# rpng/open_vins

Measured on AMD Instinct MI355X. Metric: MSCKF features/sec per EKF update (30-clone state), higher is better.
Workload: dtype f64; 1 GPU; BASELINE.json configs[2]: 2-camera radtan rig, 30-clone window, 2000 MSCKF features/update, N=248, D=208, online cam extrinsic+intrinsic calib + IMU intrinsics in the state, FEJ; features_total=2000, features_this_rank=2000, clones=30, cameras=2, state_dim=248, measurements_total=100362, parallelism=single GPU

## Files before the change

open_vins_amd/csrc/api_context.inc:

```
using namespace ovg;

static thread_local std::string g_err = "";
static int set_err(int code, const std::string &msg) {
  g_err = msg;
  return code;
}

#define HIPCHK(expr)                                                                                         \
  do {                                                                                                       \
    hipError_t _e = (expr);                                                                                  \
    if (_e != hipSuccess) {                                                                                  \
      return set_err(OVGPU_ERR_HIP, std::string(#expr) + " -> " + hipGetErrorString(_e) + " (" __FILE__ ":" + \
                                        std::to_string(__LINE__) + ")");                                     \
    }                                                                                                        \
  } while (0)

namespace {

struct AllocCount {
  std::atomic<int64_t> n{0}, bytes{0};
  void add(size_t b) { n.fetch_add(1, std::memory_order_relaxed), bytes.fetch_add((int64_t)b, std::memory_order_relaxed); }
  void sub(size_t b) { n.fetch_sub(1, std::memory_order_relaxed), bytes.fetch_sub((int64_t)b, std::memory_order_relaxed); }
};
struct DeviceAlloc {
// ... 262 lines not shown
  std::vector<int32_t> h_offsets;
  std::vector<int64_t> h_row_off;

  DevBuf<double> Hbig, gate_ws, Rws, Mt, Aaug, Yaug, dx;
  DevView<int32_t> flags;
  int W = 1;
  int64_t rows_per_node = 128;
  int tsqr_last_W = 0;
  int64_t tsqr_last_rpn = 0;
  int tsqr_last_leaf = -1;
  int tsqr_last_tree = 0;
  int tsqr_last_qh = 0;
  DevBuf<QrTreeNode> tree_nodes, tree_nodes2;
  int tree_G2 = 0;
  Stream stream2;
  Event ev_rows;
  bool gram_il = true;
  bool gram_blocks_only = false;
  bool fuse_chol_inputs = true;
  Event ev_fork, ev_join;
  DevBuf<int32_t> leaf_flags;
  int tree_overlap = -1;
  bool tree_nodes_overlap = false, tree_nodes2_overlap = false;
  DevBuf<int32_t> tree_flags;
  DevBuf<int32_t> tree_err;
  int tree_G = 0;
  bool tree_pipelined = true;
  int compress_gram = 1;
  DevBuf<double> gram_part, gram_G, gram_rho, Yaug2, Lw;
  double prior_pivot_tol = 1e-13;
  int last_route = OVGPU_COMPRESS_GRAM;
  bool whiten = true;
  bool gram_is_whitened = false;
  bool prior_on_side = false;
  int featy_skip = 0;
  DevBuf<double> fs_tq;
  DevBuf<int32_t> fs_inst;
  DevBuf<int32_t> fs_inst64;
  int inst64_D = 0;
  int feat_classes = 0;
  int64_t feat_class_batches = 0;
  int feat_class_attempt = 0;
  int last_feat_classes = 0;
  int last_class_features[4] = {0, 0, 0, 0};
  DevBuf<double> featyb_ws;
  DevBuf<double> slyb_rows, slyb_V, slyb_hq;
  DevBuf<int32_t> slyb_minfo, slyb_inst;
  int featy_big = 0;
  bool no_feat_kernel = false;
  bool raw_enable = true;
  bool gram_read_ahead = true;
  int gram_waves = 8;
  bool featy_chains = true;
  int raw_work_const = 12;
  bool raw_veto = false;
  bool raw_one_region = false;
  bool raw_cols_ok = false;
  bool raw_tables_ok = false;
  int raw_j0 = 0;
  int raw_ncls = 0, raw_ntc[RAW_MAXCLS + 1] = {0}, raw_ld[RAW_MAXCLS + 1] = {0}, raw_rcol[RAW_MAXCLS + 1] = {0};
  int64_t raw_base[RAW_MAXCLS + 1] = {0}, raw_rows[RAW_MAXCLS + 1] = {0};
  std::vector<uint8_t> h_cls_of_clone;
  DevBuf<uint8_t> cls_of_clone;
  DevBuf<int32_t> raw_featbase, raw_dst, raw_runs;
  DevBuf<double> Hraw;
  DevBuf<gram::GramRegionWG> gram_wg;
  int gram_wg_n = 0, gram_wg_tiles = 0;
  gram::GramRegionSum raw_rs;
  bool last_stack_raw = false;
  DevView<int32_t> feat_counter;
  DevBuf<int32_t> fs_minfo, fs_meas_feat, fs_pos;
  DevBuf<int32_t> fs_slots;
  std::vector<int32_t> h_order;
  std::vector<uint16_t> h_cc;
  DevBuf<double> fs_rows, fs_V, fs_z, fs_w;
  void *comm = nullptr;
  struct LoopComm *loop = nullptr;
  int comm_rank = 0, comm_world = 1;
  DevBuf<double> comm_buf;
  DevView<int32_t> chol_prog;
  DevBuf<int32_t> ctrl;
  unsigned ctrl_clean = 0;
  unsigned ctrl_pre = 0;
  DevBuf<double> chol_uinv;
  DevBuf<double> chol_wide_A, chol_wide_Y;
  bool chol_wide = true;
  int64_t chol_wide_count = 0;
  int gram_wide = 0;
  int gram_wide_on = 0;
  int64_t gram_wide_updates = 0;
  int gram_wide_attempt = 0;
  int mode_a_wide = 0;
  int mode_a_wide_on = 0;
  int64_t mode_a_wide_compressions = 0;
  int slam_mode_a = 0;
  int slam_mode_a_on = 0;
  int64_t slam_mode_a_compressions = 0;
  int mode_a_panel = 0;
  int mode_a_panel_on = 0;
  int64_t mode_a_panel_compressions = 0;
  DevBuf<double> pchol_dots;
  DevBuf<double> uinv_tiles;
  PinBuf<double> h_tri;
  int chol_slot = 0;
  bool no_chol_pipe = false;
  int tri_waves = 0;
// ... 213 lines not shown
```

open_vins_amd/csrc/api_debug.inc:

```
int ovgpu_debug_option(ovgpu_ctx *c, const char *name, int64_t value, int64_t *old_value) {
  if (!c || !name) return set_err(OVGPU_ERR_INVALID, "null argument");
  const std::string n(name);
  if (n == "chol_follow_spin_limit") {
    if (old_value) *old_value = c->chol_spin_limit;
    if (value >= 0) c->chol_spin_limit = (int)std::min<int64_t>(value, 1 << 30);
  } else if (n == "slam_chunked_fail_chunk") {
    if (old_value) *old_value = c->chunk_fail_inject;
    c->chunk_fail_inject = value >= 0 ? (int)std::min<int64_t>(value, 1 << 20) : -1;
  } else if (n == "slam_chunked_fallbacks") {
    if (old_value) *old_value = c->chunk_fallbacks;
    if (value >= 0) c->chunk_fallbacks = value;
  } else if (n == "delayed_init_fused") {
    if (old_value) *old_value = c->init_fused;
    if (value >= 0) c->init_fused = (int)std::min<int64_t>(value, 2);
  } else if (n == "delayed_init_fused_steps") {
    if (old_value) *old_value = c->init_fused_steps;
    if (value >= 0) c->init_fused_steps = value;
  } else if (n == "delayed_init_rows_steps") {
    if (old_value) *old_value = c->init_rows_steps;
    if (value >= 0) c->init_rows_steps = value;
  } else if (n == "delayed_init_fused_long") {
    if (old_value) *old_value = c->init_fused_long;
    if (value >= 0) c->init_fused_long = value != 0 ? 1 : 0;
  } else if (n == "delayed_init_long_steps") {
// ... 25 lines not shown
    if (value >= 0) c->anchored_fast = value != 0;
  } else if (n == "slam_fused") {
    if (old_value) *old_value = c->slam_fused;
    if (value >= 0) c->slam_fused = (int)std::min<int64_t>(value, 3);
  } else if (n == "slam_fused_big") {
    if (old_value) *old_value = c->slam_fused_big;
    if (value >= 0) c->slam_fused_big = (int)std::min<int64_t>(value, 1);
  } else if (n == "slam_fused_batches") {
    if (old_value) *old_value = c->slam_fused_batches;
    if (value >= 0) c->slam_fused_batches = value;
  } else if (n == "gram_blocks_only") {
    if (old_value) *old_value = c->gram_blocks_only ? 1 : 0;
    if (value >= 0) c->gram_blocks_only = value != 0;
  } else if (n == "stage_timing_period") {
    if (old_value) *old_value = c->timing_period;
    if (value >= 1) c->timing_period = (int)value, c->timing_seq = 0;
  } else if (n == "fuse_chol_inputs") {
    if (old_value) *old_value = c->fuse_chol_inputs ? 1 : 0;
    if (value >= 0) c->fuse_chol_inputs = value != 0;
  } else if (n == "featy_big") {
    if (old_value) *old_value = c->featy_big;
    if (value >= 0) c->featy_big = (int)value;
  } else if (n == "upload_kernel") {
    if (old_value) *old_value = c->up.use_kernel;
    if (value >= 0) c->up.use_kernel = c->down.use_kernel = value != 0;
  } else if (n == "upload_arena_bytes") {
    if (old_value) *old_value = (int64_t)c->up.capacity();
    if (value >= 64) c->up.want = (size_t)std::min<int64_t>(value, (int64_t)1 << 30);
  } else if (n == "upload_bypasses") {
    if (old_value) *old_value = c->up.bypasses;
    if (value >= 0) c->up.bypasses = value;
  } else if (n == "layout_every_update") {
    if (old_value) *old_value = c->layout_every_update;
    if (value >= 0) c->layout_every_update = value != 0;
  } else if (n == "tri_waves") {
    if (old_value) *old_value = c->tri_waves;
    if (value >= 0 && value <= 16) c->tri_waves = (int)value;
  } else if (n == "featy_skip") {
#ifdef OVG_FEAT_ABLATE
    if (old_value) *old_value = c->featy_skip;
    if (value >= 0) c->featy_skip = (int)value;
#else
    return set_err(OVGPU_ERR_INVALID, "featy_skip: ablation switches exist in a developer build only (-DOVG_FEAT_ABLATE)");
#endif
  } else if (n == "gram_read_ahead") {
    if (old_value) *old_value = c->gram_read_ahead ? 1 : 0;
    if (value >= 0) c->gram_read_ahead = value != 0;
  } else if (n == "gram_waves") {
    if (old_value) *old_value = c->gram_waves;
    if (value >= 0) {
      if (value != 4 && value != 8) return set_err(OVGPU_ERR_INVALID, "gram_waves: 4 or 8");
      c->gram_waves = (int)value;
    }
  } else if (n == "featy_chains") {
    if (old_value) *old_value = c->featy_chains ? 1 : 0;
    if (value >= 0) c->featy_chains = value != 0;
  } else if (n == "raw_work_const") {
    if (old_value) *old_value = c->raw_work_const;
    if (value >= 0) c->raw_work_const = (int)value;
  } else if (n == "last_stack_raw") {
    if (old_value) *old_value = c->last_stack_raw ? 1 : 0;
  } else if (n == "raw_gram_tile_rows") {
    int64_t t = 0;
    if (c->raw_tables_ok)
      for (int k = 0; k <= RAW_NEG; k++) t += c->raw_rows[k] * (int64_t)(c->raw_ntc[k] * (c->raw_ntc[k] + 1) / 2);
    if (old_value) *old_value = t;
  } else if (n == "stack_is_f32") {
    if (old_value) *old_value = c->stack_is_f32 ? 1 : 0;
  } else if (n == "last_feature_kernel") {
    if (old_value) *old_value = c->last_feat_kernel;
  } else if (n == "feat_classes") {
    if (old_value) *old_value = c->feat_classes;
    if (value >= 0) c->feat_classes = (int)std::min<int64_t>(value, 1);
  } else if (n == "feat_class_batches") {
    if (old_value) *old_value = c->feat_class_batches;
    if (value >= 0) c->feat_class_batches = value;
  } else if (n == "last_feature_classes") {
    if (old_value) *old_value = c->last_feat_classes;
  } else if (n.size() == 21 && n.compare(0, 20, "last_class_features_") == 0 && n[20] >= '0' && n[20] <= '3') {
    if (old_value) *old_value = c->last_class_features[n[20] - '0'];
  } else if (n == "last_gram_kernel") {
    if (old_value) *old_value = c->last_gram_kernel;
  } else if (n == "last_gram_workgroups") {
    if (old_value) *old_value = c->last_gram_workgroups;
  } else if (n == "last_factor_kernel") {
    if (old_value) *old_value = c->last_factor_kernel;
  } else if (n == "last_unwhiten_kernel") {
    if (old_value) *old_value = c->last_unwhiten_kernel;
  } else if (n == "chol_wide") {
    if (old_value) *old_value = c->chol_wide ? 1 : 0;
    if (value >= 0) c->chol_wide = value != 0;
  } else if (n == "chol_wide_factorisations") {
    if (old_value) *old_value = c->chol_wide_count;
    if (value >= 0) c->chol_wide_count = value;
  } else if (n == "gram_wide") {
    if (old_value) *old_value = c->gram_wide;
    if (value >= 0) c->gram_wide = (int)std::min<int64_t>(value, 1);
  } else if (n == "gram_wide_updates") {
    if (old_value) *old_value = c->gram_wide_updates;
  } else if (n == "mode_a_wide") {
    if (old_value) *old_value = c->mode_a_wide;
    if (value >= 0) c->mode_a_wide = (int)std::min<int64_t>(value, 1);
  } else if (n == "mode_a_wide_compressions") {
    if (old_value) *old_value = c->mode_a_wide_compressions;
  } else if (n == "mode_a_panel") {
    if (old_value) *old_value = c->mode_a_panel;
// ... 209 lines not shown
```

open_vins_amd/csrc/api_pipeline.inc:

```
static int enqueue_triangulate(ovgpu_ctx *c, const double *seed_pA = nullptr, const int32_t *seed_anchor = nullptr) {
  const Batch b = batch_of(c);
  if (b.F == 0) return OVGPU_OK;
  TriParams p;
  p.seed_pA = seed_pA, p.seed_anchor = seed_anchor, p.anchor_pre = c->anchor_pre.p;
  p.F = b.F, p.C = c->C, p.K = c->K;
  p.meas_offsets = b.meas_offsets, p.meas_cc = b.meas_cc, p.uvn = b.uvn, p.tab_cc = c->tab_cc.p;
  p.p_FinA = b.pA, p.p_FinG = b.pG, p.anchor_meas = c->anchor.p, p.status = b.status;
  p.opt = c->dopt;
  const size_t lds = (size_t)c->K * c->C * 12 * sizeof(double);
  if (lds > (size_t)c->lds_limit) {
    return set_err(OVGPU_ERR_CAPACITY, "k_triangulate: the pose table of K = " + std::to_string(c->K) + " cameras x C = " + std::to_string(c->C) + " clones (96 bytes a pair, " +
                                           std::to_string(lds) + " bytes) exceeds the LDS limit of " + std::to_string(c->lds_limit) + " bytes");
  }
  int wpb = c->tri_waves;
  if (wpb == 0) {
    wpb = 4;
    const int room = c->num_cu - 6;
    for (int w = 4; w <= 8 && room > 0; w *= 2) {
      const int blocks = (b.F + w - 1) / w;
      if (blocks <= room) {
        if (4 * blocks >= 3 * room) wpb = w;
        break;
      }
    }
// ... 317 lines not shown
static int enqueue_gram_factor(ovgpu_ctx *c);
static int gram_blk_row_shares(const ovgpu_ctx *c, int NT, int64_t nchunks) {
  int shares = c->num_cu;
  if (NT > gram::GR_NT_BLK) shares = std::max(1, c->num_cu / (gram::GR_NT_WIDE / gram::GB_T * (gram::GR_NT_WIDE / gram::GB_T + 1) / 2));
  return (int)std::max<int64_t>(1, std::min<int64_t>(shares, nchunks));
}
static size_t gram_part_doubles(const ovgpu_ctx *c, int NT, int64_t nchunks) {
  const size_t G = (size_t)std::max<int64_t>(1, std::min<int64_t>(c->num_cu, nchunks));
  size_t need = NT <= gram::GR_NT_BLK ? G * (size_t)(NT * (NT + 1) / 2) * 256 : 0;
  if (NT > gram::GR_NT || c->gram_fp32) {
    const size_t NB = (size_t)(NT + gram::GB_T - 1) / gram::GB_T, pairs = NB * (NB + 1) / 2;
    need = std::max(need, pairs * (size_t)gram_blk_row_shares(c, NT, nchunks) * gram::GB_T * gram::GB_T * 256);
  }
  return need;
}
static int gram_route_tile_cap(const ovgpu_ctx *c) { return c->gram_wide_on >= 1 && c->whiten && !c->gram_fp32 ? gram::GR_NT_WIDE : gram::GR_NT_BLK; }
static int mode_a_tile_cap(const ovgpu_ctx *c) { return c->mode_a_wide_on >= 1 && c->whiten && !c->gram_fp32 ? gram::GR_NT_WIDE : gram::GR_NT_BLK; }
constexpr int MODE_A_PANEL_MIN_NT = 17;
static bool mode_a_panel_factor(const ovgpu_ctx *c, int NTf) { return c->mode_a_panel_on >= 1 && NTf >= MODE_A_PANEL_MIN_NT && NTf <= gram::GR_NT_BLK; }
static int enqueue_compress_gram(ovgpu_ctx *c, bool factor = true) {
  const int D = c->D, LD = c->LD, NT = (LD + 15) / 16, NP = NT * (NT + 1) / 2, LG = 16 * NT;
  const int64_t rows_total = batch_of(c).rows_total;
  const int64_t nchunks = (rows_total + gram::GR_ROWS - 1) / gram::GR_ROWS;
  const int G = (int)std::max<int64_t>(1, std::min<int64_t>(c->num_cu, nchunks));
  if (NT <= gram::GR_NT_BLK) HIPCHK(c->gram_part.reserve((size_t)G * NP * 256));
  HIPCHK(c->gram_G.reserve((size_t)LG * LG));
  if (c->stack_is_f32) {
    const int LDF = c->stack_ldf, NTM = LDF / 32, P = gram32::gram32_parts(NTM), slots = P * gram32::G32_NW * gram32::G32_MAXT;
    if (c->gram32_ntm != NTM || c->gram32_P != P) {
      std::vector<int32_t> tab((size_t)slots);
      gram32::gram32_tile_table(NTM, P, tab.data());
      HIPCHK(c->gram32_tiles.reserve((size_t)slots));
      HIPCHK(hipMemcpyAsync(c->gram32_tiles.p, tab.data(), sizeof(int32_t) * slots, hipMemcpyHostToDevice, c->stream));
      HIPCHK(upload_sync(c, c->stream));
      c->gram32_ntm = NTM, c->gram32_P = P;
    }
    const int64_t by_rows = (rows_total + gram32::G32_ROWS_WG - 1) / gram32::G32_ROWS_WG;
    const int64_t by_cus = std::min<int64_t>((2 * c->num_cu + P - 1) / P, (rows_total + 127) / 128);
    const int Gw = (int)std::max<int64_t>(1, std::max(by_rows, by_cus));
    HIPCHK(c->gram32_part.reserve((size_t)P * Gw * gram32::G32_NW * gram32::G32_MAXT * 1024));
    gram32::Gram32Params q;
    q.H = c->Hbig32.p, q.part = c->gram32_part.p, q.tiles = c->gram32_tiles.p, q.rows_total = rows_total, q.LDF = LDF, q.LD = LD;
    hipLaunchKernelGGL(with_max_lds<gram32::k_gram_f32>(c), dim3(Gw, P), dim3(gram32::G32_NTH), gram32::gram32_lds_bytes(LDF), c->stream, q);
    hipLaunchKernelGGL(gram32::k_gram_f32_reduce, dim3(slots, 4), dim3(256), 0, c->stream, (const int32_t *)c->gram32_tiles.p, Gw,
                       (const float *)c->gram32_part.p, c->gram_G.p, LG);
    HIPCHK(hipGetLastError());
    c->last_gram_kernel = 5, c->last_gram_workgroups = Gw;
    return factor ? set_err(OVGPU_ERR_CAPACITY, "the fp32 Gram variant feeds the on-device update only") : OVGPU_OK;
  }
  if (c->last_stack_raw) {
    HIPCHK(c->gram_part.reserve((size_t)std::max(c->gram_wg_tiles, 1) * 256));
    const int waves = c->gram_read_ahead ? c->gram_waves : 4;
    const auto kern = !c->gram_read_ahead ? with_max_lds<gram::k_gram_regions<false>>(c)
                      : waves == 8        ? with_max_lds<gram::k_gram_regions<true, 8>>(c)
                                          : with_max_lds<gram::k_gram_regions<true>>(c);
    hipLaunchKernelGGL(kern, dim3(c->gram_wg_n), dim3(64 * waves), gram::gram_lds_bytes(), c->stream, (const double *)c->Hraw.p, (const gram::GramRegionWG *)c->gram_wg.p,
                       c->gram_part.p);
    hipLaunchKernelGGL(gram::k_gram_regions_reduce, dim3(NP, 256 / gram::RR_E), dim3(gram::RR_E * gram::RR_G), 0, c->stream, NT, D, c->raw_rs,
                       (const gram::GramRegionWG *)c->gram_wg.p, c->gram_wg_n, (const double *)c->gram_part.p, c->gram_G.p);
    HIPCHK(hipGetLastError());
    c->last_gram_kernel = 4;
    return factor ? enqueue_gram_factor(c) : OVGPU_OK;
  }
  gram::GramParams g;
  g.LD = LD, g.NT = NT, g.rows_total = rows_total, g.H = c->Hbig.p, g.part = c->gram_part.p;
  if (NT == gram::GR_NT + 7 && !c->gram_fp32 && !c->gram_blocks_only) {
    const int Gw = G;
    hipLaunchKernelGGL(with_max_lds<gram::k_gram_wide_top<7>>(c), dim3(Gw), dim3(256), gram::gram_wide_top_lds_bytes(), c->stream, g);
    hipLaunchKernelGGL(with_max_lds<gram::k_gram_wide_win<7>>(c), dim3(Gw), dim3(256), gram::gram_lds_bytes(), c->stream, g);
    hipLaunchKernelGGL(gram::k_gram_reduce, dim3(NP), dim3(1024), 0, c->stream, NT, Gw, c->gram_part.p, c->gram_G.p);
    HIPCHK(hipGetLastError());
    c->last_gram_kernel = 3;
    return factor ? enqueue_gram_factor(c) : OVGPU_OK;
  }
  if (NT > gram::GR_NT || c->gram_fp32) {
    const int NB = (NT + gram::GB_T - 1) / gram::GB_T, pairs = NB * (NB + 1) / 2;
    const int Gb = gram_blk_row_shares(c, NT, nchunks);
    HIPCHK(c->gram_part.reserve((size_t)pairs * Gb * gram::GB_T * gram::GB_T * 256));
    g.part = c->gram_part.p;
    if (!c->gram_fp32) hipLaunchKernelGGL(with_max_lds<gram::k_gram_blk<false>>(c), dim3(Gb, pairs), dim3(256), gram::gram_blk_lds_bytes(), c->stream, g, NB);
    else hipLaunchKernelGGL(with_max_lds<gram::k_gram_blk<true>>(c), dim3(Gb, pairs), dim3(256), gram::gram_blk_lds_bytes() / 2, c->stream, g, NB);
    hipLaunchKernelGGL(gram::k_gram_blk_reduce, dim3(gram::GB_T * gram::GB_T, pairs), dim3(256), 0, c->stream, NB, NT, Gb, c->gram_part.p, c->gram_G.p);
    HIPCHK(hipGetLastError());
    c->last_gram_kernel = 2, c->last_gram_workgroups = Gb;
    return factor ? enqueue_gram_factor(c) : OVGPU_OK;
  }
  switch ((NT + 1) / 2) {
  case 1: launch_gram<2>(c, G, g, c->stream, c->gram_il); break;
  case 2: launch_gram<4>(c, G, g, c->stream, c->gram_il); break;
  case 3: launch_gram<6>(c, G, g, c->stream, c->gram_il); break;
  case 4: launch_gram<8>(c, G, g, c->stream, c->gram_il); break;
  case 5: launch_gram<10>(c, G, g, c->stream, c->gram_il); break;
  case 6: launch_gram<12>(c, G, g, c->stream, c->gram_il); break;
  case 7: launch_gram<14>(c, G, g, c->stream, c->gram_il); break;
  default:
    if (NT == 15) launch_gram<15>(c, G, g, c->stream, c->gram_il);
    else launch_gram<16>(c, G, g, c->stream, c->gram_il);
    break;
  }
  hipLaunchKernelGGL(gram::k_gram_reduce, dim3(NP), dim3(1024), 0, c->stream, NT, G, c->gram_part.p, c->gram_G.p);
  HIPCHK(hipGetLastError());
  c->last_gram_kernel = 1;
  return factor ? enqueue_gram_factor(c) : OVGPU_OK;
}

static int enqueue_gram_factor(ovgpu_ctx *c) {
  const int D = c->D, LD = c->LD, LG = 16 * ((LD + 15) / 16);
// ... 809 lines not shown
```

open_vins_amd/csrc/api_state.inc:

```

const char *ovgpu_last_error(void) { return g_err.c_str(); }

void ovgpu_default_options(ovgpu_options *o) {
  if (!o) return;
  std::memset(o, 0, sizeof(*o));
  o->chi2_multipler = 5.0, o->sigma_pix = 1.0;
  o->triangulate_1d = 0, o->refine_features = 1, o->max_runs = 5;
  o->init_lamda = 1e-3, o->max_lamda = 1e10, o->min_dx = 1e-6, o->min_dcost = 1e-6, o->lam_mult = 10;
  o->min_dist = 0.10, o->max_dist = 60, o->max_baseline = 40, o->max_cond_number = 10000;
  o->do_fej = 1, o->do_calib_camera_pose = 1, o->do_calib_camera_intrinsics = 1;
  o->feat_rep_msckf = OVGPU_REP_GLOBAL_3D;
}

double ovgpu_chi2_quantile_95(int dof) { return chi2_quantile_95(dof); }
int ovgpu_abi_version(void) { return OVGPU_ABI_VERSION; }

static int init_context(ovgpu_ctx *c, const ovgpu_options *opts, int device) {
  c->device = device;
  c->opts = *opts;
  hipDeviceProp_t prop;
  HIPCHK(hipGetDeviceProperties(&prop, device));
  c->num_cu = prop.multiProcessorCount > 0 ? prop.multiProcessorCount : 256;
  c->lds_limit = (int)std::min<size_t>(prop.sharedMemPerBlock, 160 * 1024);
  HIPCHK(hipStreamCreateWithFlags(&c->stream.h, hipStreamNonBlocking));
// ... 590 lines not shown
  if (!c->raw_enable || !c->raw_cols_ok || F <= 0 || M <= 0 || n <= 0) return OVGPU_OK;
  std::vector<int32_t> fb((size_t)F * RAW_MAXCLS, 0);
  int64_t run[RAW_MAXCLS + 1] = {0};
  for (int f = 0; f < F; f++) {
    int cnt[RAW_MAXCLS] = {0};
    for (int i = b.h_offsets[f]; i < b.h_offsets[f + 1]; i++) cnt[c->h_cls_of_clone[anchor_clone(cc[i])]]++;
    int below = 0;
    for (int k = 0; k < n; k++) {
      fb[(size_t)f * RAW_MAXCLS + k] = (int32_t)(run[k] - 2 * below);
      run[k] += 2 * cnt[k], below += cnt[k];
    }
  }
  run[RAW_NEG] = (int64_t)4 * F;
  int64_t total = 0;
  double work[RAW_MAXCLS + 1] = {0}, work_sum = 0;
  int live = 0;
  for (int k = 0; k <= RAW_NEG; k++) {
    if (k >= n && k != RAW_NEG) {
      c->raw_rows[k] = 0, c->raw_base[k] = total;
      continue;
    }
    if (run[k] >= ((int64_t)1 << RAW_CLS_SHIFT)) return OVGPU_OK;
    c->raw_rows[k] = run[k], c->raw_base[k] = total;
    total += run[k] * c->raw_ld[k];
    work[k] = (double)run[k] * (0.5 * c->raw_ntc[k] * (c->raw_ntc[k] + 1) + (double)c->raw_work_const);
    work_sum += work[k], live += run[k] > 0;
  }
  HIPCHK(c->Hraw.reserve((size_t)std::max<int64_t>(total, 1)));
  HIPCHK(c->raw_featbase.reserve(fb.size()));
  HIPCHK(c->raw_dst.reserve((size_t)M));
  HIPCHK(c->raw_runs.reserve((size_t)F * feat::FY_RUNREC * 4));
  HIPCHK(c->up.put(c->raw_featbase.p, fb.data(), sizeof(int32_t) * fb.size()));
  const int G = std::max(c->num_cu, live);
  int wgs[RAW_MAXCLS + 1] = {0}, given = 0;
  for (int k = 0; k <= RAW_NEG; k++)
    if (c->raw_rows[k] > 0) wgs[k] = std::max(1, (int)std::floor(work[k] / work_sum * (G - live)) + 1), given += wgs[k];
  for (int k = RAW_NEG; given > G && k >= 0; k = k > 0 ? k - 1 : RAW_NEG)
    if (wgs[k] > 1) wgs[k]--, given--;
  std::vector<gram::GramRegionWG> tab;
  int tiles = 0;
  c->raw_rs.n = 0;
  for (int k = 0; k <= RAW_NEG; k++) {
    if (wgs[k] == 0) continue;
    const int64_t nchunks = (c->raw_rows[k] + gram::GR_ROWS - 1) / gram::GR_ROWS;
    const int w = (int)std::min<int64_t>(wgs[k], nchunks);
    {
      const int q = c->raw_rs.n++;
      c->raw_rs.ntc[q] = c->raw_ntc[k], c->raw_rs.rcol[q] = c->raw_rcol[k];
    }
    for (int j = 0; j < w; j++) {
      gram::GramRegionWG r;
      r.ntc = c->raw_ntc[k], r.ld = c->raw_ld[k], r.rcol = c->raw_rcol[k], r.pad = 0;
      if (r.ld > 16 * r.ntc) return set_err(OVGPU_ERR_INVALID, "raw_stack_layout: a region's row stride exceeds its tile columns");
      r.h_off = c->raw_base[k], r.rows = c->raw_rows[k];
      r.chunk_begin = (int)((nchunks * j) / w), r.chunk_end = (int)((nchunks * (j + 1)) / w);
      r.part_tile = tiles, r.region = (c->raw_rs.n - 1) | (k == RAW_NEG ? 16 : 0);
      tiles += r.ntc * (r.ntc + 1) / 2;
      tab.push_back(r);
    }
  }
  c->gram_wg_n = (int)tab.size(), c->gram_wg_tiles = tiles;
  HIPCHK(c->gram_wg.reserve(tab.size()));
  HIPCHK(c->up.put(c->gram_wg.p, tab.data(), sizeof(gram::GramRegionWG) * tab.size()));
  c->raw_tables_ok = true;
  return OVGPU_OK;
}

static int begin_feature_batch(ovgpu_ctx *c, int F, int M, const int32_t *offsets) {
  c->have_feats = false, c->tri_readable = false;
  c->raw_tables_ok = false;
  int m_max = 0;
  for (int f = 0; f < F; f++) {
    const int m = offsets[f + 1] - offsets[f];
    if (m < 0) return set_err(OVGPU_ERR_INVALID, "meas_offsets not monotone");
    m_max = std::max(m_max, m);
  }
  c->F = F, c->M = M, c->m_max = m_max;
  c->have_feat_sigma = c->have_feat_mult = false;
  c->h_feat_lm.clear(), c->h_feat_rep.clear();
  c->h_offsets.assign(offsets, offsets + (F > 0 ? F + 1 : 0));
  if (F == 0) c->h_offsets.assign(1, 0);

  const int need = std::max(500, 2 * m_max + 1);
  if ((int)c->h_chi2_table.size() < need) {
    const int old = (int)c->h_chi2_table.size();
    c->h_chi2_table.resize(need, 0.0);
    for (int i = std::max(old, 1); i < need; i++) c->h_chi2_table[i] = chi2_quantile_95(i);
  }
  c->chi2_table_len = (int)c->h_chi2_table.size();
  HIPCHK(c->chi2_table.reserve(c->chi2_table_len));

  HIPCHK(c->meas_offsets.reserve(F + 1));
  HIPCHK(c->meas_cc.reserve(M));
  HIPCHK(c->uv.reserve((size_t)2 * M));
  HIPCHK(c->uvn.reserve((size_t)2 * M));
  HIPCHK(c->pA.reserve((size_t)3 * F));
  HIPCHK(c->pG.reserve((size_t)3 * F));
  HIPCHK(c->chi2.reserve(F));
  HIPCHK(c->chi2_thr.reserve(F));
  HIPCHK(c->anchor.reserve(F));
  HIPCHK(c->anchor_pre.reserve(F));
  HIPCHK(c->status.reserve(F));

  std::vector<int32_t> order(std::max(F, 1), 0);
  track_order(offsets, F, m_max, order.data());
  c->h_order.assign(order.begin(), order.begin() + F);
// ... 66 lines not shown
```

open_vins_amd/csrc/k_gram.h:

```cpp
#pragma once
#include <hip/hip_runtime.h>
#include <stdint.h>
#include <type_traits>
#include <utility>

namespace ovg {
namespace gram {

typedef double d4 __attribute__((ext_vector_type(4)));

constexpr int GR_ROWS = 32;
constexpr int GR_LS = 272;
constexpr int GR_NT = 16;
constexpr int GR_NT_BLK = 24;
constexpr int GR_NT_WIDE = 32;

struct GramParams {
  int LD, NT;
  int64_t rows_total;
  const double *H;
  double *part;
};

__host__ __device__ inline int pair_index(int NT, int ti, int tj) { return ti * NT - (ti * (ti - 1)) / 2 + (tj - ti); }
// ... 384 lines not shown
        __builtin_amdgcn_sched_barrier(0);
#ifdef OVG_GRAM_PROF
        GRAM_T(w0)
        __builtin_amdgcn_s_waitcnt(0xC07F | ((NU - 1) << 8));
        GRAM_T(w1)
        prof_wait += w1 - w0;
#endif
      }
      static_for(std::make_integer_sequence<int, NS>{}, [&](auto sc) {
        constexpr int s = decltype(sc)::value;
        constexpr bool ahead = ks < 7 && s < NU, slot = s < SL && (ks & 3) * SL + s < NQ;
        if constexpr (s < N) {
          constexpr int ti = D::row_of(T0 + s), tj = D::col_of(T0 + s);
          GRAM_MFMA(bb[ks & 1][ti], bb[ks & 1][tj], acc[s]);
        }
        if constexpr (ahead || slot) __builtin_amdgcn_sched_barrier(0);
        if constexpr (ahead) {
          constexpr int j = D::nth_col(W, s);
          bb[(ks + 1) & 1][j] = rowp[4 * GR_LS + 16 * j];
        }
        if constexpr (slot) {
          constexpr int q = (ks & 3) * SL + s;
          if constexpr (ks < 4) put(nxt, q);
          else fetch1(q);
        }
        if constexpr (ahead || slot) __builtin_amdgcn_sched_barrier(0);
      });
      __builtin_amdgcn_sched_barrier(0);
    });
    left_v = left_f;
#ifdef OVG_GRAM_PROF
    GRAM_T(b0)
#endif
    asm volatile("s_waitcnt lgkmcnt(0)\n\ts_barrier" ::: "memory");
#ifdef OVG_GRAM_PROF
    GRAM_T(b1)
    prof_bar += b1 - b0;
#endif
  }
#ifdef OVG_GRAM_PROF
  GRAM_T(prof_t2)
  if (lane == 0) {
    long long *o = gram_prof_buf + ((size_t)(blockIdx.x & 1023) * 8 + W) * 8;
    o[3] = prof_t1 - prof_t0, o[4] = prof_t2 - prof_t1, o[5] = prof_wait, o[6] = prof_bar;
  }
#endif
#pragma unroll
  for (int s = 0; s < N; s++) {
    double2 *o = reinterpret_cast<double2 *>(p.part + (size_t)(T0 + s) * 256) + lane;
    o[0] = double2{acc[s][0], acc[s][1]}, o[64] = double2{acc[s][2], acc[s][3]};
  }
}

template <int NTC, bool PF, int NW> __device__ __forceinline__ void gram_region_body(const GramParams &p, double *gram_lds, int tid, int lane, int wave, int cb, int ce) {
  if constexpr (NW == 8) {
    switch (wave) {
    case 0: gram_w8<0, NTC>(p, gram_lds, tid, lane, cb, ce); break;
    case 1: gram_w8<1, NTC>(p, gram_lds, tid, lane, cb, ce); break;
    case 2: gram_w8<2, NTC>(p, gram_lds, tid, lane, cb, ce); break;
    case 3: gram_w8<3, NTC>(p, gram_lds, tid, lane, cb, ce); break;
    case 4: gram_w8<4, NTC>(p, gram_lds, tid, lane, cb, ce); break;
    case 5: gram_w8<5, NTC>(p, gram_lds, tid, lane, cb, ce); break;
    case 6: gram_w8<6, NTC>(p, gram_lds, tid, lane, cb, ce); break;
    default: gram_w8<7, NTC>(p, gram_lds, tid, lane, cb, ce); break;
    }
  } else {
    d4 acc[GR_ACC];
#pragma unroll
    for (int i = 0; i < GR_ACC; i++) acc[i] = d4{0, 0, 0, 0};
    switch (wave) {
    case 0: gram_il_loop<0, NTC, true, PF>(p, gram_lds, tid, lane, cb, ce, acc), gram_put<0, true>(p.part, NTC, lane, acc); break;
    case 1: gram_il_loop<1, NTC, true, PF>(p, gram_lds, tid, lane, cb, ce, acc), gram_put<1, true>(p.part, NTC, lane, acc); break;
    case 2: gram_il_loop<2, NTC, true, PF>(p, gram_lds, tid, lane, cb, ce, acc), gram_put<2, true>(p.part, NTC, lane, acc); break;
    default: gram_il_loop<3, NTC, true, PF>(p, gram_lds, tid, lane, cb, ce, acc), gram_put<3, true>(p.part, NTC, lane, acc); break;
    }
  }
}
template <bool PF, int NW = 4> __global__ void __launch_bounds__(64 * NW) k_gram_regions(const double *H, const GramRegionWG *tab, double *part) {
  static_assert(NW == 4 || (NW == 8 && PF), "the eight-wavefront form reads ahead");
  extern __shared__ double gram_lds[];
  const int tid = threadIdx.x, lane = tid & 63, wave = tid >> 6;
  const GramRegionWG r = tab[blockIdx.x];
#ifdef OVG_GRAM_PROF
  const long long prof_w0 = wall_clock64();
  GRAM_T(prof_c0)
#endif
  for (int i = tid, w = 16 * r.ntc - r.ld; i < 2 * GR_ROWS * w; i += 64 * NW) gram_lds[(i / w) * GR_LS + r.ld + i % w] = 0.0;
  __syncthreads();
#ifdef OVG_GRAM_PROF
  GRAM_T(prof_c1)
#endif
  GramParams p;
  p.LD = r.ld, p.NT = r.ntc, p.rows_total = r.rows, p.H = H + r.h_off, p.part = part + (size_t)r.part_tile * 256;
  switch (r.ntc) {
  case 4: gram_region_body<4, PF, NW>(p, gram_lds, tid, lane, wave, r.chunk_begin, r.chunk_end); break;
  case 6: gram_region_body<6, PF, NW>(p, gram_lds, tid, lane, wave, r.chunk_begin, r.chunk_end); break;
  case 8: gram_region_body<8, PF, NW>(p, gram_lds, tid, lane, wave, r.chunk_begin, r.chunk_end); break;
  case 10: gram_region_body<10, PF, NW>(p, gram_lds, tid, lane, wave, r.chunk_begin, r.chunk_end); break;
  case 12: gram_region_body<12, PF, NW>(p, gram_lds, tid, lane, wave, r.chunk_begin, r.chunk_end); break;
  case 14: gram_region_body<14, PF, NW>(p, gram_lds, tid, lane, wave, r.chunk_begin, r.chunk_end); break;
  default: gram_region_body<15, PF, NW>(p, gram_lds, tid, lane, wave, r.chunk_begin, r.chunk_end); break;
  }
#ifdef OVG_GRAM_PROF
  __builtin_amdgcn_s_waitcnt(0x0070);
  GRAM_T(prof_c2)
  if (lane == 0) {
    long long *o = gram_prof_buf + ((size_t)(blockIdx.x & 1023) * 8 + wave) * 8;
    o[0] = prof_w0, o[1] = wall_clock64(), o[2] = prof_c1 - prof_c0, o[7] = (prof_c2 - prof_c1) - o[3] - o[4];
  }
#endif
}

struct GramRegionSum {
  int32_t n;
  int32_t ntc[9], rcol[9];
};
constexpr int RR_E = 64, RR_G = 16, RR_U = 16;
__global__ void __launch_bounds__(RR_E *RR_G) k_gram_regions_reduce(int NT, int D, GramRegionSum rs, const GramRegionWG *__restrict__ tab, int total, const double *__restrict__ part,
                                                                        double *__restrict__ G) {
  __shared__ int eoff[9][RR_E];
  __shared__ double tot[RR_G][RR_E];
  const int LG = 16 * NT;
  const int idx = blockIdx.x, e = threadIdx.x & (RR_E - 1), t = RR_E * blockIdx.y + e;
  const int grp = __builtin_amdgcn_readfirstlane(threadIdx.x / RR_E);
  int ti = 0, rem = idx;
  while (rem >= NT - ti) rem -= NT - ti, ti++;
  const int tj = ti + rem;
  const int q = 2 * (t >> 7) + (t & 1), lane = (t >> 1) & 63;
  const int i = 16 * ti + 4 * q + (lane >> 4), j = 16 * tj + (lane & 15);
  if (grp < rs.n) {
    const int rc = rs.rcol[grp], ntc = rs.ntc[grp];
    int li = i == D ? rc : (i < rc && i < D ? i : -1), lj = j == D ? rc : (j < rc && j < D ? j : -1);
    int off = -1;
    if (li >= 0 && lj >= 0) {
      if ((li >> 4) > (lj >> 4)) {
        const int x = li;
        li = lj, lj = x;
      }
      const int lq = (li & 15) >> 2, llane = 16 * (li & 3) + (lj & 15);
      off = pair_index(ntc, li >> 4, lj >> 4) * 256 + (lq >> 1) * 128 + 2 * llane + (lq & 1);
    }
    eoff[grp][e] = off;
  }
  __syncthreads();
  double s = 0.0;
  for (int base = 0; base < total; base += RR_G * RR_U) {
    int ptile[RR_U], reg[RR_U];
#pragma unroll
    for (int u = 0; u < RR_U; u++) {
      const int f = base + grp + RR_G * u, fc = f < total ? f : total - 1;
      ptile[u] = tab[fc].part_tile, reg[u] = f < total ? tab[fc].region : -1;
    }
    double a[RR_U];
    bool ok[RR_U];
// ... 552 lines not shown
```

Baseline: 2.973 million features/s.

## Stage Gram input tiles into LDS with direct global-to-LDS loads in a ring

Adds an eight-wavefront Gram kernel variant that copies raw Jacobian chunks from global memory straight into a multi-slot LDS ring buffer using global_load_lds, then synchronises with vmcnt-based barriers. The aim is to overlap the next chunks' loads with MFMA work and skip the register round-trip of staging through VGPRs. Padding columns now read from a shared zero slot instead of zeroing LDS pad regions. It becomes the default and adds layout checks for even base and row counts, which could reject layouts that were accepted before.

```diff
diff --git a/open_vins_amd/csrc/api_context.inc b/open_vins_amd/csrc/api_context.inc
--- a/open_vins_amd/csrc/api_context.inc
+++ b/open_vins_amd/csrc/api_context.inc
@@ -338,6 +338,7 @@
   bool gram_read_ahead = true;
   int gram_waves = 8;
   bool featy_chains = true;
+  int gram_stage_dma = 1;
   int raw_work_const = 12;
   bool raw_veto = false;
   bool raw_one_region = false;
diff --git a/open_vins_amd/csrc/api_debug.inc b/open_vins_amd/csrc/api_debug.inc
--- a/open_vins_amd/csrc/api_debug.inc
+++ b/open_vins_amd/csrc/api_debug.inc
@@ -101,6 +101,13 @@
       if (value != 4 && value != 8) return set_err(OVGPU_ERR_INVALID, "gram_waves: 4 or 8");
       c->gram_waves = (int)value;
     }
+  } else if (n == "gram_stage_dma") {
+    if (old_value) *old_value = c->gram_stage_dma;
+    if (value >= 0) {
+      if (value == 2) return set_err(OVGPU_ERR_INVALID, "gram_stage_dma: the padded image (2) is not built");
+      if (value > 1) return set_err(OVGPU_ERR_INVALID, "gram_stage_dma: 0 or 1");
+      c->gram_stage_dma = (int)value;
+    }
   } else if (n == "featy_chains") {
     if (old_value) *old_value = c->featy_chains ? 1 : 0;
     if (value >= 0) c->featy_chains = value != 0;
diff --git a/open_vins_amd/csrc/api_pipeline.inc b/open_vins_amd/csrc/api_pipeline.inc
--- a/open_vins_amd/csrc/api_pipeline.inc
+++ b/open_vins_amd/csrc/api_pipeline.inc
@@ -393,7 +393,7 @@
     HIPCHK(c->gram_part.reserve((size_t)std::max(c->gram_wg_tiles, 1) * 256));
     const int waves = c->gram_read_ahead ? c->gram_waves : 4;
     const auto kern = !c->gram_read_ahead ? with_max_lds<gram::k_gram_regions<false>>(c)
-                      : waves == 8        ? with_max_lds<gram::k_gram_regions<true, 8>>(c)
+                      : waves == 8        ? (c->gram_stage_dma == 1 ? with_max_lds<gram::k_gram_regions<true, 8, 1>>(c) : with_max_lds<gram::k_gram_regions<true, 8>>(c))
                                           : with_max_lds<gram::k_gram_regions<true>>(c);
     hipLaunchKernelGGL(kern, dim3(c->gram_wg_n), dim3(64 * waves), gram::gram_lds_bytes(), c->stream, (const double *)c->Hraw.p, (const gram::GramRegionWG *)c->gram_wg.p,
                        c->gram_part.p);
diff --git a/open_vins_amd/csrc/api_state.inc b/open_vins_amd/csrc/api_state.inc
--- a/open_vins_amd/csrc/api_state.inc
+++ b/open_vins_amd/csrc/api_state.inc
@@ -666,6 +666,8 @@
       gram::GramRegionWG r;
       r.ntc = c->raw_ntc[k], r.ld = c->raw_ld[k], r.rcol = c->raw_rcol[k], r.pad = 0;
       if (r.ld > 16 * r.ntc) return set_err(OVGPU_ERR_INVALID, "raw_stack_layout: a region's row stride exceeds its tile columns");
+      if ((c->raw_base[k] & 1) || (c->raw_rows[k] & 1)) return set_err(OVGPU_ERR_INVALID, "raw_stack_layout: a region's base or row count is no multiple of two doubles");
+      if (r.ld <= 16 * (r.ntc - 2)) return set_err(OVGPU_ERR_INVALID, "raw_stack_layout: a region's rows end before its last two tile columns");
       r.h_off = c->raw_base[k], r.rows = c->raw_rows[k];
       r.chunk_begin = (int)((nchunks * j) / w), r.chunk_end = (int)((nchunks * (j + 1)) / w);
       r.part_tile = tiles, r.region = (c->raw_rs.n - 1) | (k == RAW_NEG ? 16 : 0);
diff --git a/open_vins_amd/csrc/k_gram.h b/open_vins_amd/csrc/k_gram.h
--- a/open_vins_amd/csrc/k_gram.h
+++ b/open_vins_amd/csrc/k_gram.h
@@ -460,8 +460,165 @@
   }
 }
 
-template <int NTC, bool PF, int NW> __device__ __forceinline__ void gram_region_body(const GramParams &p, double *gram_lds, int tid, int lane, int wave, int cb, int ce) {
-  if constexpr (NW == 8) {
+constexpr int GR_LDS_DOUBLES = 2 * GR_ROWS * GR_LS;
+constexpr int GR_RING_MAX = 8;
+constexpr int GR_ZERO = GR_LDS_DOUBLES - 2;
+__device__ __forceinline__ void gram_dma16(const double *src, double *dst_wave) {
+  __builtin_amdgcn_global_load_lds((const __attribute__((address_space(1))) void *)src, (__attribute__((address_space(3))) void *)dst_wave, 16, 0, 0);
+}
+template <int LO, int HI> __device__ __forceinline__ void gram_dma_barrier(int n) {
+  if constexpr (LO == HI) {
+    asm volatile("s_waitcnt vmcnt(%0) lgkmcnt(0)\n\ts_barrier" ::"n"(LO) : "memory");
+  } else {
+    constexpr int MID = (LO + HI) / 2;
+    if (n <= MID) gram_dma_barrier<LO, MID>(n);
+    else gram_dma_barrier<MID + 1, HI>(n);
+  }
+}
+__host__ __device__ constexpr int gram_ring_depth(int ntc) {
+  const int n = GR_ZERO / (GR_ROWS * 16 * ntc);
+  return n < GR_RING_MAX ? n : GR_RING_MAX;
+}
+
+template <int W, int NTC> __device__ __forceinline__ void gram_w8_dma(const GramParams &p, double *gram_lds, int tid, int lane, int chunk_begin, int chunk_end) {
+  using D = Deal8<NTC>;
+  constexpr int T0 = D::begin(W), N = D::count(W), NU = D::ncols(W);
+  constexpr int NQ = (NTC + 1) / 2;
+  constexpr int NS = N > NU ? N : NU;
+  constexpr bool PAD1 = (D::cols(W) >> (NTC - 1)) & 1, PAD2 = (D::cols(W) >> (NTC - 2)) & 1;
+  constexpr int NB = gram_ring_depth(NTC), MAXN = (NB - 2) * NQ;
+  static_assert(NB >= 2 && MAXN < 64, "two buffers at least; the VM counter holds the loads in flight");
+  const int LD = p.LD, stage_d = GR_ROWS * LD, nch = 16 * LD;
+  const int g = lane >> 4, cl = lane & 15;
+  d4 acc[N];
+#pragma unroll
+  for (int i = 0; i < N; i++) acc[i] = d4{0, 0, 0, 0};
+  const bool pad1 = 16 * (NTC - 1) + cl >= LD, pad2 = 16 * (NTC - 2) + cl >= LD;
+  const double *const zero1 = gram_lds + GR_ZERO - 16 * (NTC - 1), *const zero2 = gram_lds + GR_ZERO - 16 * (NTC - 2);
+  const int last = (int)((p.rows_total - 1) / GR_ROWS);
+  const int nv_last = (int)((p.rows_total - (int64_t)last * GR_ROWS) / 2) * LD;
+  auto count_w = [&](int nv) {
+    const int n = (nv - 64 * W + 511) >> 9;
+    return n < 0 ? 0 : (n > NQ ? NQ : n);
+  };
+  const int n_full = count_w(nch), n_last = count_w(nv_last);
+  int rq_nv = 0;
+  const double *rq_src = p.H;
+  double *rq_dst = gram_lds;
+  auto aim = [&](int t, int slot) {
+    rq_nv = t >= chunk_end ? 0 : (t == last ? nv_last : nch);
+    rq_src = p.H + (int64_t)(t < chunk_end ? t : chunk_begin) * stage_d + 2 * (64 * W + lane);
+    rq_dst = gram_lds + slot * stage_d + 128 * W;
+    if (rq_nv > 0 && rq_nv < nch) {
+#pragma unroll
+      for (int q = 0; q < NQ; q++) {
+        const int c = 64 * W + 512 * q + lane;
+        if (c >= rq_nv && c < nch) *reinterpret_cast<double2 *>(rq_dst + 1024 * q + 2 * lane) = double2{0.0, 0.0};
+      }
+    }
+  };
+  auto piece = [&](int q) {
+    if (64 * W + 512 * q + lane < rq_nv) gram_dma16(rq_src + 1024 * q, rq_dst + 1024 * q);
+  };
+  auto beyond = [&](int s1) {
+    const int hi = s1 + NB - 2 < chunk_end - 1 ? s1 + NB - 2 : chunk_end - 1, cnt = hi - s1;
+    return cnt <= 0 ? 0 : cnt * n_full - (hi == last ? n_full - n_last : 0);
+  };
+#ifdef OVG_GRAM_PROF
+  long long prof_wait = 0, prof_bar = 0;
+  GRAM_T(prof_t0)
+#endif
+  for (int i = 0; i < NB - 1; i++) {
+    aim(chunk_begin + i, i);
+#pragma unroll
+    for (int q = 0; q < NQ; q++) piece(q);
+  }
+  gram_dma_barrier<0, MAXN>(beyond(chunk_begin));
+#ifdef OVG_GRAM_PROF
+  GRAM_T(prof_t1)
+#endif
+  double bb[2][GR_NT];
+  int cs = 0;
+  for (int chunk = chunk_begin; chunk < chunk_end; chunk++) {
+    const double *cur = gram_lds + cs * stage_d;
+    aim(chunk + NB - 1, cs == 0 ? NB - 1 : cs - 1);
+    __builtin_amdgcn_sched_barrier(0);
+    static_for(std::make_integer_sequence<int, 8>{}, [&](auto kc) {
+      constexpr int ks = decltype(kc)::value;
+      if constexpr (ks == 0) {
+        const double *r0 = cur + g * LD + cl, *r1 = PAD1 && pad1 ? zero1 : r0, *r2 = PAD2 && pad2 ? zero2 : r0;
+        static_for(std::make_integer_sequence<int, NU>{}, [&](auto n) {
+          constexpr int j = D::nth_col(W, decltype(n)::value);
+          bb[0][j] = (j == NTC - 1 ? r1 : j == NTC - 2 ? r2 : r0)[16 * j];
+        });
+        __builtin_amdgcn_sched_barrier(0);
+#ifdef OVG_GRAM_PROF
+        GRAM_T(w0)
+        __builtin_amdgcn_s_waitcnt(0xC07F | ((NU - 1) << 8));
+        GRAM_T(w1)
+        prof_wait += w1 - w0;
+#endif
+      }
+      const double *rn = cur + (4 * (ks + 1) + g) * LD + cl, *rn1 = PAD1 && pad1 ? zero1 : rn, *rn2 = PAD2 && pad2 ? zero2 : rn;
+      static_for(std::make_integer_sequence<int, NS>{}, [&](auto sc) {
+        constexpr int s = decltype(sc)::value;
+        constexpr bool ahead = ks < 7 && s < NU;
+        if constexpr (s < N) {
+          constexpr int ti = D::row_of(T0 + s), tj = D::col_of(T0 + s);
+          GRAM_MFMA(bb[ks & 1][ti], bb[ks & 1][tj], acc[s]);
+        }
+        if constexpr (s == 0 && 2 * ks < NQ) {
+          __builtin_amdgcn_sched_barrier(0);
+          piece(2 * ks);
+          if constexpr (2 * ks + 1 < NQ) piece(2 * ks + 1);
+          __builtin_amdgcn_sched_barrier(0);
+        }
+        if constexpr (ahead) {
+          constexpr int j = D::nth_col(W, s);
+          __builtin_amdgcn_sched_barrier(0);
+          bb[(ks + 1) & 1][j] = (j == NTC - 1 ? rn1 : j == NTC - 2 ? rn2 : rn)[16 * j];
+          __builtin_amdgcn_sched_barrier(0);
+        }
+      });
+      __builtin_amdgcn_sched_barrier(0);
+    });
+#ifdef OVG_GRAM_PROF
+    GRAM_T(b0)
+#endif
+    gram_dma_barrier<0, MAXN>(beyond(chunk + 1));
+#ifdef OVG_GRAM_PROF
+    GRAM_T(b1)
+    prof_bar += b1 - b0;
+#endif
+    cs = cs + 1 == NB ? 0 : cs + 1;
+  }
+#ifdef OVG_GRAM_PROF
+  GRAM_T(prof_t2)
+  if (lane == 0) {
+    long long *o = gram_prof_buf + ((size_t)(blockIdx.x & 1023) * 8 + W) * 8;
+    o[3] = prof_t1 - prof_t0, o[4] = prof_t2 - prof_t1, o[5] = prof_wait, o[6] = prof_bar;
+  }
+#endif
+#pragma unroll
+  for (int s = 0; s < N; s++) {
+    double2 *o = reinterpret_cast<double2 *>(p.part + (size_t)(T0 + s) * 256) + lane;
+    o[0] = double2{acc[s][0], acc[s][1]}, o[64] = double2{acc[s][2], acc[s][3]};
+  }
+}
+
+template <int NTC, bool PF, int NW, int DMA = 0> __device__ __forceinline__ void gram_region_body(const GramParams &p, double *gram_lds, int tid, int lane, int wave, int cb, int ce) {
+  if constexpr (NW == 8 && DMA == 1) {
+    switch (wave) {
+    case 0: gram_w8_dma<0, NTC>(p, gram_lds, tid, lane, cb, ce); break;
+    case 1: gram_w8_dma<1, NTC>(p, gram_lds, tid, lane, cb, ce); break;
+    case 2: gram_w8_dma<2, NTC>(p, gram_lds, tid, lane, cb, ce); break;
+    case 3: gram_w8_dma<3, NTC>(p, gram_lds, tid, lane, cb, ce); break;
+    case 4: gram_w8_dma<4, NTC>(p, gram_lds, tid, lane, cb, ce); break;
+    case 5: gram_w8_dma<5, NTC>(p, gram_lds, tid, lane, cb, ce); break;
+    case 6: gram_w8_dma<6, NTC>(p, gram_lds, tid, lane, cb, ce); break;
+    default: gram_w8_dma<7, NTC>(p, gram_lds, tid, lane, cb, ce); break;
+    }
+  } else if constexpr (NW == 8) {
     switch (wave) {
     case 0: gram_w8<0, NTC>(p, gram_lds, tid, lane, cb, ce); break;
     case 1: gram_w8<1, NTC>(p, gram_lds, tid, lane, cb, ce); break;
@@ -484,8 +641,9 @@
     }
   }
 }
-template <bool PF, int NW = 4> __global__ void __launch_bounds__(64 * NW) k_gram_regions(const double *H, const GramRegionWG *tab, double *part) {
+template <bool PF, int NW = 4, int DMA = 0> __global__ void __launch_bounds__(64 * NW) k_gram_regions(const double *H, const GramRegionWG *tab, double *part) {
   static_assert(NW == 4 || (NW == 8 && PF), "the eight-wavefront form reads ahead");
+  static_assert(DMA == 0 || (DMA == 1 && NW == 8), "the DMA form is the eight-wavefront kernel's");
   extern __shared__ double gram_lds[];
   const int tid = threadIdx.x, lane = tid & 63, wave = tid >> 6;
   const GramRegionWG r = tab[blockIdx.x];
@@ -493,7 +651,11 @@
   const long long prof_w0 = wall_clock64();
   GRAM_T(prof_c0)
 #endif
-  for (int i = tid, w = 16 * r.ntc - r.ld; i < 2 * GR_ROWS * w; i += 64 * NW) gram_lds[(i / w) * GR_LS + r.ld + i % w] = 0.0;
+  if constexpr (DMA == 1) {
+    if (tid < 2) gram_lds[GR_ZERO + tid] = 0.0;
+  } else {
+    for (int i = tid, w = 16 * r.ntc - r.ld; i < 2 * GR_ROWS * w; i += 64 * NW) gram_lds[(i / w) * GR_LS + r.ld + i % w] = 0.0;
+  }
   __syncthreads();
 #ifdef OVG_GRAM_PROF
   GRAM_T(prof_c1)
@@ -501,13 +663,13 @@
   GramParams p;
   p.LD = r.ld, p.NT = r.ntc, p.rows_total = r.rows, p.H = H + r.h_off, p.part = part + (size_t)r.part_tile * 256;
   switch (r.ntc) {
-  case 4: gram_region_body<4, PF, NW>(p, gram_lds, tid, lane, wave, r.chunk_begin, r.chunk_end); break;
-  case 6: gram_region_body<6, PF, NW>(p, gram_lds, tid, lane, wave, r.chunk_begin, r.chunk_end); break;
-  case 8: gram_region_body<8, PF, NW>(p, gram_lds, tid, lane, wave, r.chunk_begin, r.chunk_end); break;
-  case 10: gram_region_body<10, PF, NW>(p, gram_lds, tid, lane, wave, r.chunk_begin, r.chunk_end); break;
-  case 12: gram_region_body<12, PF, NW>(p, gram_lds, tid, lane, wave, r.chunk_begin, r.chunk_end); break;
-  case 14: gram_region_body<14, PF, NW>(p, gram_lds, tid, lane, wave, r.chunk_begin, r.chunk_end); break;
-  default: gram_region_body<15, PF, NW>(p, gram_lds, tid, lane, wave, r.chunk_begin, r.chunk_end); break;
+  case 4: gram_region_body<4, PF, NW, DMA>(p, gram_lds, tid, lane, wave, r.chunk_begin, r.chunk_end); break;
+  case 6: gram_region_body<6, PF, NW, DMA>(p, gram_lds, tid, lane, wave, r.chunk_begin, r.chunk_end); break;
+  case 8: gram_region_body<8, PF, NW, DMA>(p, gram_lds, tid, lane, wave, r.chunk_begin, r.chunk_end); break;
+  case 10: gram_region_body<10, PF, NW, DMA>(p, gram_lds, tid, lane, wave, r.chunk_begin, r.chunk_end); break;
+  case 12: gram_region_body<12, PF, NW, DMA>(p, gram_lds, tid, lane, wave, r.chunk_begin, r.chunk_end); break;
+  case 14: gram_region_body<14, PF, NW, DMA>(p, gram_lds, tid, lane, wave, r.chunk_begin, r.chunk_end); break;
+  default: gram_region_body<15, PF, NW, DMA>(p, gram_lds, tid, lane, wave, r.chunk_begin, r.chunk_end); break;
   }
 #ifdef OVG_GRAM_PROF
   __builtin_amdgcn_s_waitcnt(0x0070);
```

Result: no change. 2.984 million features/s (median of 6 runs) (+0.4%).
